# musket-ml/segmentation_training_pipeline

Measured on AMD Instinct MI355X. Metric: images/sec U-Net/ResNet34 512x512 bs16 training step, higher is better.
Workload: dtype bf16; 1 GPU; U-Net/ResNet34 512x512x3 1-class, batch 16 per GPU, BCE+Dice, Adam, on-device augment S1 (BASELINE.json configs[1]); global_batch=16, parallelism=dp1, hipgraph=True

## Files before the change

segmentation_training_pipeline_amd/csrc/conv_common.h:

```cpp
#pragma once
#include <type_traits>
#include "common.h"
#include <cstdlib>

struct ConvArgs {
  const char* src0;
  const char* src1;
  const char* weight;
  const char* residual;
  const float* bias;
  char* dst0;
  char* dst1;
  int N, Hs0, Ws0, Hv, Wv, C0, C1, Ctot, mode;
  int KH, KW, stride, pad, Ho, Wo, Cout, Cd0, Cd1;
  int acc0, acc1, relu;
  int K, P, HoWo, wrows;
  int ntile_m, ntile_n;
  uint32_t bytes0, bytes1, bytesw;
  float* stats;
  int stat_slots;
  BnBack bnb;
  BnBack pbn;
  FastDiv divC, divKW, divHoWo, divWo, divNtm;
  int zperm, zPc, zH2W2, zW2, zcpt;
  FastDiv divPc, divH2W2, divW2, divCpt;
  const char* weight_up;
  uint32_t byteswu;
  int upc, ucpt0, ucpt1;
  FastDiv divU0, divU1;
  const char* fold_src;
  const char* fold_weight;
  int fold_cpt;
  uint32_t bytes_fold, bytesw_fold;
  int no_rm;
  int ep_generic;
  int sum2x2;
  float* sg_out;
  unsigned* sg_cnt;
  int sg_G;
  int d2s;
};

__device__ __forceinline__ void stats_store(const ConvArgs& a, size_t idx, float v) {
  if (a.sg_out) __hip_atomic_store(a.stats + idx, v, __ATOMIC_RELAXED, __HIP_MEMORY_SCOPE_AGENT);
  else a.stats[idx] = v;
}
template <int NT>
__device__ __forceinline__ void stats_group_finish(const ConvArgs& a, int Cs, int cout0, int nch, int tile_m, int tile_n, int ntile, int tid,
                                                   unsigned* word) {
  if (!a.sg_out) return;
  const int G = a.sg_G, g = tile_n / G, ngroups = (ntile + G - 1) / G;
  const int members = (ntile - g * G) < G ? (ntile - g * G) : G;
  unsigned* const cnt = a.sg_cnt + (size_t)tile_m * ngroups + g;
  asm volatile("s_waitcnt vmcnt(0)" ::: "memory");
  __syncthreads();
  if (tid == 0) *word = __hip_atomic_fetch_add(cnt, 1u, __ATOMIC_RELAXED, __HIP_MEMORY_SCOPE_AGENT);
  __syncthreads();
  if (*word != (unsigned)(members - 1)) return;
  if (tid == 0) __hip_atomic_store(cnt, 0u, __ATOMIC_RELAXED, __HIP_MEMORY_SCOPE_AGENT);
  for (int r = tid; r < 2 * nch; r += NT) {
    const int stat = r / nch, ch = cout0 + (r - stat * nch);
    if (ch >= Cs) continue;
    const float* col = a.stats + ((size_t)stat * Cs + ch) * ntile + (size_t)g * G;
    float v[16];
#pragma unroll
    for (int j = 0; j < 16; ++j) v[j] = j < members ? __hip_atomic_load(col + j, __ATOMIC_RELAXED, __HIP_MEMORY_SCOPE_AGENT) : 0.f;
    float sum = v[0];
#pragma unroll
    for (int j = 1; j < 16; ++j) sum += v[j];
    a.sg_out[((size_t)stat * Cs + ch) * ngroups + g] = sum;
  }
}
static inline int stats_group_size(int cols) {
  if (cols <= 128) return 0;
// ... 419 lines not shown
  if (p->Cd0 <= 0 || p->Cd0 > p->Cout || (p->Cd0 < p->Cout && (!p->dst1 || (p->Cd0 & 3) || ((p->Cout - p->Cd0) & 3))))
    return STP_E_BADARG;
  if (p->N <= 0 || p->Ho <= 0 || p->Wo <= 0 || p->Cout <= 0 || p->KH <= 0 || p->KW <= 0 || p->stride <= 0) return STP_E_BADARG;
  a.src0 = (const char*)p->src0; a.src1 = (const char*)p->src1; a.weight = (const char*)p->weight;
  a.residual = (const char*)p->residual; a.bias = p->bias; a.dst0 = (char*)p->dst0; a.dst1 = (char*)p->dst1;
  a.N = p->N; a.Hs0 = p->Hs0; a.Ws0 = p->Ws0; a.Hv = p->Hv; a.Wv = p->Wv; a.C0 = p->C0; a.C1 = p->C1;
  a.Ctot = p->C0 + p->C1; a.mode = p->src0_mode;
  a.KH = p->KH; a.KW = p->KW; a.stride = p->stride; a.pad = p->pad; a.Ho = p->Ho; a.Wo = p->Wo;
  a.Cout = p->Cout; a.Cd0 = p->Cd0; a.Cd1 = p->Cout - p->Cd0;
  a.acc0 = p->accumulate0; a.acc1 = p->accumulate1; a.relu = p->relu;
  a.K = p->KH * p->KW * a.Ctot;
  const int64_t P = (int64_t)p->N * p->Ho * p->Wo;
  if (P >= (1ll << 31)) return STP_E_BADARG;
  a.P = (int)P; a.HoWo = p->Ho * p->Wo; a.wrows = round_up(p->Cout, 16);
  a.divC = make_fastdiv((uint32_t)a.Ctot); a.divKW = make_fastdiv((uint32_t)a.KW);
  a.divHoWo = make_fastdiv((uint32_t)(p->Ho * p->Wo)); a.divWo = make_fastdiv((uint32_t)p->Wo);
  const int64_t lim = 1ll << 31;
  const int64_t b0 = (int64_t)p->N * p->Hs0 * p->Ws0 * p->C0 * sz;
  const int64_t b1 = (int64_t)p->N * p->Hv * p->Wv * p->C1 * sz;
  const int64_t bw = (int64_t)a.wrows * a.K * sz;
  a.bytes0 = (uint32_t)(b0 < lim ? b0 : 0); a.bytes1 = (uint32_t)(b1 < lim ? b1 : 0); a.bytesw = (uint32_t)(bw < lim ? bw : 0);
  a.ntile_m = a.ntile_n = 0;
  a.zperm = 0;
  a.weight_up = (const char*)p->weight_up; a.byteswu = 0; a.upc = 0; a.ucpt0 = a.ucpt1 = 1;
  a.fold_src = a.fold_weight = nullptr; a.fold_cpt = 0; a.bytes_fold = a.bytesw_fold = 0;
  {
    static const int no_rm = (getenv("STP_IGEMM_RM") && atoi(getenv("STP_IGEMM_RM")) == 0) ? 1 : 0;
    a.no_rm = no_rm;
    static const int ep_generic = (getenv("STP_EPILOGUE_SPECIAL") && atoi(getenv("STP_EPILOGUE_SPECIAL")) == 0) ? 1 : 0;
    a.ep_generic = ep_generic;
  }
  a.stats = p->stats_partial;
  a.stat_slots = p->stats_slots;
  if (a.stats && ((p->Cout & 3) || (p->Cd0 != p->Cout && !p->dst_sum2x2))) return STP_E_BADARG;
  a.sum2x2 = p->dst_sum2x2 ? 1 : 0;
  a.sg_out = nullptr; a.sg_cnt = nullptr; a.sg_G = 0;
  a.d2s = p->s2d_dgrad ? 1 : 0;
  if (p->stats_group > 1) {
    if (!p->stats_group_out || !p->stats_group_counters || !a.stats || a.stat_slots || p->stats_group > 16 || (p->stats_group & (p->stats_group - 1)))
      return STP_E_BADARG;
    a.sg_out = p->stats_group_out; a.sg_cnt = p->stats_group_counters; a.sg_G = p->stats_group;
  }
  if (a.stat_slots && (!a.stats || (a.stat_slots & (a.stat_slots - 1)) || a.stat_slots > 64)) return STP_E_BADARG;
  a.bnb.x = (const char*)p->bnb_x; a.bnb.mean = p->bnb_mean; a.bnb.rstd = p->bnb_rstd; a.bnb.gamma = p->bnb_gamma;
  a.bnb.beta = p->bnb_beta; a.bnb.relu = p->bnb_relu;
  a.pbn.x = nullptr; a.pbn.mean = p->src_bn_mean; a.pbn.rstd = p->src_bn_rstd; a.pbn.gamma = p->src_bn_gamma; a.pbn.beta = p->src_bn_beta;
  a.pbn.relu = p->src_bn_relu;
  *c4_out = c4;
  *ut_out = 0;
  if (!c4 && b0 < lim && b1 < lim && bw < lim) {
    if ((a.Ctot % ke == 0) && (a.C0 % ke == 0)) *ut_out = 1;
    else if (a.C1 == 0 && (ke % a.Ctot == 0)) *ut_out = 2;
  }
  return STP_OK;
}
```

segmentation_training_pipeline_amd/csrc/conv_halo.hip:

```cpp
#include "conv_common.h"
#include <cstdlib>
#include <type_traits>

#define STP_OOB 0x80000000u
#define HALO_NWST 4
#if defined(STP_TIMING_REAL)
#define STP_CLOCK() __builtin_amdgcn_s_memrealtime()
#else
#define STP_CLOCK() __builtin_amdgcn_s_memtime()
#endif


__device__ __forceinline__ void wait_vmcnt_n(int n) {
  switch (n) {
    case 0: wait_vmcnt<0>(); break;
    case 1: wait_vmcnt<1>(); break;
    case 2: wait_vmcnt<2>(); break;
    case 3: wait_vmcnt<3>(); break;
    case 4: wait_vmcnt<4>(); break;
    case 5: wait_vmcnt<5>(); break;
    case 6: wait_vmcnt<6>(); break;
    case 7: wait_vmcnt<7>(); break;
    case 8: wait_vmcnt<8>(); break;
    case 9: wait_vmcnt<9>(); break;
// ... 572 lines not shown
#pragma unroll
      for (int dx = 0; dx < 3; ++dx)
#pragma unroll
        for (int kc = 0; kc < 4; ++kc) b_lane[dx][kc] += d;
    }
    if (!grp_b) __builtin_amdgcn_s_barrier();
  }
  STP_STAMP(2);

  epilogue_rm<TH, BM, WM, WN, EP>(a, acc, smem, n, y0, x0, cout0, tile_n, wm, wn, lane, tid, wave);
#if defined(STP_TIMING)
  asm volatile("s_waitcnt vmcnt(0)" ::: "memory");
  STP_STAMP(3);
  if (tid == 0)
    for (int i = 0; i < 4; ++i) tdbg[(size_t)blockIdx.x * 4 + i] = tstamp[i];
#endif
#endif
}

#define HALO_MIN_WAVES(TH, BM) ((TH) == 16 && (BM) == 64 ? 4 : 1)
template <int TH, int BM, int WM, int WN, int EP>
__global__ __launch_bounds__(512, HALO_MIN_WAVES(TH, BM)) void conv_halo_kernel(const ConvArgs a) { conv_halo_body<TH, BM, WM, WN, EP, false, false>(a); }
template <int TH, int BM, int WM, int WN, int EP>
__global__ __launch_bounds__(512, HALO_MIN_WAVES(TH, BM)) void conv_halo_pbn_kernel(const ConvArgs a) { conv_halo_body<TH, BM, WM, WN, EP, true, false>(a); }
template <int TH, int BM, int WM, int WN, int EP>
__global__ __launch_bounds__(512, 1) void conv_halo_r6_kernel(const ConvArgs a) { conv_halo_body<TH, BM, WM, WN, EP, false, false, 9, false, 6>(a); }
template <int TH, int BM, int WM, int WN, int EP>
__global__ __launch_bounds__(512, HALO_MIN_WAVES(TH, BM)) void conv_halo2_kernel(const ConvArgs a) { conv_halo_body<TH, BM, WM, WN, EP, false, true>(a); }
template <int TH, int BM, int WM, int WN, int EP>
__global__ __launch_bounds__(512, HALO_MIN_WAVES(TH, BM)) void conv_halo_fold1_kernel(const ConvArgs a) { conv_halo_body<TH, BM, WM, WN, EP, false, true, 9, true>(a); }
template <int TH, int BM, int WM, int WN, int EP>
__global__ __launch_bounds__(512, HALO_MIN_WAVES(TH, BM)) void conv_halo_s2d_kernel(const ConvArgs a) { conv_halo_body<TH, BM, WM, WN, EP, false, true, 4>(a); }

#if !defined(STP_P64_STAGGER)
#define STP_P64_STAGGER 4
#endif
template <int TH, int BM, int WM, int WN, int EP>
__global__ __launch_bounds__(256, 2) void conv_halo_p64_kernel(const ConvArgs a_in) {
  static_assert(TH == 8 && BM == 64 && WM == 2 && WN == 2 && EP <= 2, "the 64 -> 64 form");
#if defined(__HIP_DEVICE_COMPILE__)
#if defined(STP_TIMING)
  ConvArgs a = a_in;
  unsigned long long* const tdbg = reinterpret_cast<unsigned long long*>(const_cast<float*>(a_in.bias));
  a.bias = nullptr;
  unsigned long long tsum[4] = {0, 0, 0, 0}, tlast = STP_CLOCK();
  const unsigned long long tfirst = tlast;
#define P64_LAP(i) { const unsigned long long now_ = STP_CLOCK(); tsum[i] += now_ - tlast; tlast = now_; }
#else
  const ConvArgs& a = a_in;
#define P64_LAP(i)
#endif
  typedef bf16_t T;
  constexpr int NTH = 256;
  constexpr int TW = 16, HWD = TW + 2, HH = TH + 2, NHP = HH * HWD;
  constexpr int SROWS = (NHP + 7) / 8 * 8, SLAB = SROWS * 128;
  constexpr int NPASS = (SROWS + 31) / 32;
  constexpr int RW = TH / WN, TN = RW / 2;
  constexpr int PF = 2;
  extern __shared__ __attribute__((aligned(16))) char smem[];
  char* const stage = smem + 2 * SLAB;
  const int tid = threadIdx.x, lane = tid & 63;
  const int wave = __builtin_amdgcn_readfirstlane(tid >> 6);
  const int wm = wave / WN, wn = wave % WN;
  const int l15 = lane & 15, l31 = lane & 31, l4b = (lane >> 4) & 1, l5 = lane >> 5;
  const int ntile = a.ntile_n, nwg = gridDim.x;
  const int wg = xcd_remap(blockIdx.x, nwg);
// ... 145 lines not shown
    done = true;
  }
  hipLaunchKernelGGL(kern, dim3(a.ntile_m * a.ntile_n), dim3(512), lds, s, a);
  STP_LAUNCH_CHECK();
  return STP_OK;
}

template <int TH, int BM, int WM, int WN>
static int launch_halo(ConvArgs& a, hipStream_t s) {
  if (a.sum2x2) return launch_halo_ep<TH, BM, WM, WN, 3>(a, s);
  if (a.bnb.x) return launch_halo_ep<TH, BM, WM, WN, 2>(a, s);
  if (a.stats) return launch_halo_ep<TH, BM, WM, WN, 1>(a, s);
  return launch_halo_ep<TH, BM, WM, WN, 0>(a, s);
}

static bool halo2_enabled() {
  static const bool on = !(getenv("STP_HALO2") && atoi(getenv("STP_HALO2")) == 0);
  return on;
}
static bool halo_src_ok(const stp_conv_params* p) {
  const bool direct = p->src0_mode == STP_SRC_DIRECT && p->Hs0 == p->Hv && p->Ws0 == p->Wv;
  if (direct && p->C1 == 0) return true;
  const bool up2 = p->src0_mode == STP_SRC_NEAREST2X && p->Hs0 * 2 == p->Hv && p->Ws0 * 2 == p->Wv;
  return halo2_enabled() && (direct || up2) && (p->C1 == 0 || (p->src1 && (p->C1 % 64) == 0)) && !p->src_bn_mean && !p->bnb_x && !p->dst_sum2x2 &&
         p->Cd0 == p->Cout;
}
static bool halo_s2d_ok(const stp_conv_params* p) {
  static const bool on = !(getenv("STP_S2D") && atoi(getenv("STP_S2D")) == 0);
  return on && p && p->s2d_dgrad && p->dtype == STP_H16 && p->KH == 2 && p->KW == 2 && p->stride == 1 && p->pad == 0 && p->src0_mode == STP_SRC_DIRECT &&
         p->Hs0 == p->Hv && p->Ws0 == p->Wv && p->Ho == p->Hv && p->Wo == p->Wv && (p->Wo % 16) == 0 && (p->Ho % 8) == 0 && p->C0 >= 64 &&
         (p->C0 % 64) == 0 && (p->C1 == 0 || (p->src1 && p->fold_weight && (p->C1 % 64) == 0)) && (p->Cout % 128) == 0 && p->Cd0 == p->Cout && !p->dst1 &&
         !p->dst_sum2x2 && !p->stats_slots && !p->src_bn_mean && !p->bias && !p->relu && !p->residual && !p->accumulate1;
}
static bool halo_fold1_ok(const stp_conv_params* p) {
  static const bool on = !(getenv("STP_FOLD1") && atoi(getenv("STP_FOLD1")) == 0);
  return on && p->fold_src && p->fold_weight && p->fold_C >= 64 && (p->fold_C % 64) == 0 && p->C1 == 0 && p->src0_mode == STP_SRC_DIRECT &&
         !p->src_bn_mean && !p->dst_sum2x2 && !p->dst1 && p->Cd0 == p->Cout && !p->bias && !p->relu && !p->residual;
}
static bool halo_p64_ok(const stp_conv_params* p) {
  static const bool on = !(getenv("STP_HALO_P64") && atoi(getenv("STP_HALO_P64")) == 0);
  return on && p->C0 == 64 && p->C1 == 0 && p->Cout == 64 && p->Cd0 == 64 && !p->dst1 && p->src0_mode == STP_SRC_DIRECT && !p->fold_src && !p->s2d_dgrad &&
         !p->src_bn_mean && !p->dst_sum2x2 && (p->Ho % 8) == 0;
}
static int halo_cus() {
  static int n = 0;
  if (!n) {
    int dev = 0, v = 0;
    if (hipGetDevice(&dev) != hipSuccess || hipDeviceGetAttribute(&v, hipDeviceAttributeMultiprocessorCount, dev) != hipSuccess || v <= 0) v = 256;
    n = v;
  }
  return n;
}
template <int EP>
static int launch_halo_p64_ep(ConvArgs& a, hipStream_t s) {
  constexpr int TH = 8, NHP = (TH + 2) * 18, SROWS = (NHP + 7) / 8 * 8;
  const size_t lds = (size_t)2 * SROWS * 128 + (size_t)TH * 16 * (64 * 4 + 16);
  static_assert(2 * SROWS * 128 + TH * 16 * (64 * 4 + 16) >= 9 * 64 * 128, "the weight image fits the workgroup's LDS");
  a.ntile_m = 1;
  a.ntile_n = a.N * (a.Ho / TH) * (a.Wo / 16);
  auto kern = conv_halo_p64_kernel<8, 64, 2, 2, EP>;
  static bool attr_set = false;
  if (!attr_set) {
    if (hipFuncSetAttribute(reinterpret_cast<const void*>(kern), hipFuncAttributeMaxDynamicSharedMemorySize, 160 * 1024) != hipSuccess) return STP_E_LAUNCH;
    attr_set = true;
  }
  const int slots = 2 * halo_cus();
  const int nwg = a.ntile_n < slots ? a.ntile_n : slots;
  hipLaunchKernelGGL(kern, dim3(nwg), dim3(256), lds, s, a);
  STP_LAUNCH_CHECK();
  return STP_OK;
}
static int launch_halo_p64(ConvArgs& a, hipStream_t s) {
  if (a.sum2x2 || a.pbn.mean) return STP_E_BADARG;
  if (a.bnb.x) return launch_halo_p64_ep<2>(a, s);
  if (a.stats) return launch_halo_p64_ep<1>(a, s);
  return launch_halo_p64_ep<0>(a, s);
}

static bool halo_shape_ok(const stp_conv_params* p) {
  if (p && p->s2d_dgrad) return halo_s2d_ok(p);
  if (p && p->fold_src && !halo_fold1_ok(p)) return false;
  return p && p->dtype == STP_H16 && p->KH == 3 && p->KW == 3 && p->stride == 1 && p->pad == 1 && halo_src_ok(p) &&
         p->C0 >= 64 && (p->C0 % 64) == 0 && p->Ho == p->Hv && p->Wo == p->Wv &&
         (p->Wo % 16) == 0 && (p->Ho % 8) == 0 && (p->Cout % 16) == 0 && p->Cout >= 64 && !p->stats_slots &&
         (!p->dst_sum2x2 || (p->bnb_x && (p->Cd0 % 64) == 0 && !p->bias && !p->relu && !p->residual &&
                             (p->Cd0 == p->Cout || (p->dst1 && p->Cd0 < p->Cout)))) &&
         (p->Cd0 % 8) == 0 &&
         (!p->src_bn_mean || (p->src_bn_rstd && p->C0 <= 512));
}

static int halo_auto(const stp_conv_params* p) {
  if (!halo_shape_ok(p)) return -1;
  {
    static const int force = getenv("STP_HALO_FORCE") ? atoi(getenv("STP_HALO_FORCE")) : -1;
    if (force >= 0 && force < 4 && (p->Ho % (force == 0 || force == 2 ? 16 : 8)) == 0) return force;
  }
  const int64_t px16 = (p->Ho % 16) == 0 ? (int64_t)p->N * (p->Ho / 16) * (p->Wo / 16) : 0;
  const int64_t px8 = (int64_t)p->N * (p->Ho / 8) * (p->Wo / 16);
  if (p->s2d_dgrad) {
    const int ct2 = ceil_div(p->Cout, 128);
    if (px16 * ct2 >= 256) return 0;
    return px8 * ct2 >= 192 ? 1 : -1;
  }
  if (p->C1 > 0 || p->src0_mode != STP_SRC_DIRECT) {
    static const bool c64 = !(getenv("STP_HALO2_64") && atoi(getenv("STP_HALO2_64")) == 0);
    if (p->Cout <= 64 && !c64) return -1;
  }
  if (p->fold_src && p->C0 == 64) {
    return px8 * ceil_div(p->Cout, 64) >= 512 ? 3 : -1;
  }
  if (p->C0 == 64 && p->C1 == 0) {
    if (p->Cout > 64 && (p->Ho % 32) == 0 && (int64_t)p->N * (p->Ho / 32) * (p->Wo / 16) * ceil_div(p->Cout, 64) >= 512) return 4;
    static const int p64 = getenv("STP_HALO_P64") ? atoi(getenv("STP_HALO_P64")) : 0;
    if (p64 == 1 && halo_p64_ok(p) && px8 >= 4 * halo_cus()) return 5;
    static const int v4 = getenv("STP_HALO_64V4") ? atoi(getenv("STP_HALO_64V4")) : 0;
    if (v4 == 1 && (p->Ho % 32) == 0 && (int64_t)p->N * (p->Ho / 32) * (p->Wo / 16) >= 512) return 4;
    if (px16 * ceil_div(p->Cout, 64) >= 512) return 2;
    if (px8 * ceil_div(p->Cout, 64) >= 512) return 3;
    return -1;
  }
  const int ct = ceil_div(p->Cout, 128);
  if (p->Cout > 64 && px16 * ct >= 256) return 0;
  if (p->Cout > 64 && px8 * ct >= 192) return 1;
  if (px8 * ceil_div(p->Cout, 64) >= 192) return 3;
  return -1;
}

extern "C" int stp_conv2d_halo_variant(const stp_conv_params* p) {
  if (!p) return -1;
  int v = -1;
  if (p->tile >= STP_TILE_HALO && p->tile < STP_TILE_HALO + HALO_NCFG) {
    v = p->tile - STP_TILE_HALO;
    if (!halo_shape_ok(p) || (p->Ho % HALO_CFGS[v].th) || (v == 4 && (p->C0 != 64 || p->C1)) || (p->s2d_dgrad && v > 1) || (v == 5 && !halo_p64_ok(p))) return -1;
  } else if (p->tile == 0) {
    v = halo_auto(p);
  }
  if (v >= 0 && p->dst_sum2x2 && (p->Cd0 % HALO_CFGS[v].bm)) return -1;
  return v;
}

extern "C" int stp_conv2d_halo_tiles(const stp_conv_params* p, int variant) {
  return p->N * (p->Ho / HALO_CFGS[variant].th) * (p->Wo / 16);
}

extern "C" int stp_conv2d_halo(const stp_conv_params* p, int variant, void* stream) {
  if (variant < 0 || variant >= HALO_NCFG || !halo_shape_ok(p) || (p->Ho % HALO_CFGS[variant].th) || (variant == 4 && (p->C0 != 64 || p->C1)) ||
      (p->s2d_dgrad && variant > 1) || (variant == 5 && !halo_p64_ok(p))) return STP_E_BADARG;
  ConvArgs a;
  bool c4;
  int ut;
  const int rc = fill_args(p, a, &c4, &ut);
  if (rc != STP_OK) return rc;
  if (ut != 1) return STP_E_BADARG;
  if (a.bnb.x && (!a.stats || !a.bnb.mean || !a.bnb.rstd || p->relu || p->residual)) return STP_E_BADARG;
  if (a.sum2x2 && (!a.bnb.x || (p->Cd0 % HALO_CFGS[variant].bm))) return STP_E_BADARG;
  if (!p->s2d_dgrad && p->fold_src) {
    if (!halo_fold1_ok(p)) return STP_E_BADARG;
    const int64_t bf = (int64_t)p->N * p->Hv * p->Wv * p->fold_C * 2, bwf = (int64_t)round_up(p->Cout, 16) * p->fold_C * 2;
    if (bf >= (1ll << 31) || bwf >= (1ll << 31)) return STP_E_BADARG;
    a.src1 = (const char*)p->fold_src; a.C1 = p->fold_C; a.Ctot = a.C0 + a.C1; a.bytes1 = (uint32_t)bf;
    a.fold_weight = (const char*)p->fold_weight; a.bytesw_fold = (uint32_t)bwf;
  }
  if (p->s2d_dgrad) {
    const int64_t rows = round_up(p->Cout / 4, 16), bw = rows * 9 * p->C0 * 2, bf = rows * (int64_t)p->C1 * 2;
    if (bw >= (1ll << 31) || bf >= (1ll << 31) || (p->C1 > 0 && !p->fold_weight)) return STP_E_BADARG;
    a.bytesw = (uint32_t)bw;
    a.fold_weight = p->C1 > 0 ? (const char*)p->fold_weight : nullptr;
    a.bytesw_fold = (uint32_t)bf;
  }
  const_cast<stp_conv_params*>(p)->stats_tiles = stp_conv2d_halo_tiles(p, variant) * (p->s2d_dgrad ? 4 : 1);
  hipStream_t s = (hipStream_t)stream;
  switch (variant) {
    case 0: return launch_halo<16, 128, 2, 4>(a, s);
    case 1: return launch_halo<8, 128, 2, 4>(a, s);
    case 2: return launch_halo<16, 64, 1, 8>(a, s);
    case 3: return launch_halo<8, 64, 2, 4>(a, s);
    case 4: return launch_halo<32, 64, 1, 8>(a, s);
    case 5: return launch_halo_p64(a, s);
    default: return STP_E_BADARG;
  }
}
```

segmentation_training_pipeline_amd/csrc/conv_igemm.hip:

```cpp
#include "conv_common.h"
#include <cstdlib>

#define STP_OOB 0x80000000u

template <typename T, int BM, int BN, int WM, int WN, int STAGES, bool UNI, bool UPC = false, bool ZP = false>
__global__ __launch_bounds__(256) void conv_igemm_ut_kernel(const ConvArgs a) {
  static_assert(!UPC || ZP, "the class-collapsed layers use the parity-class pixel order");
  static_assert(WM * WN == 4 && BM % 16 == 0 && BN % 32 == 0 && STAGES >= 2, "config");
#if defined(__HIP_DEVICE_COMPILE__)
  constexpr int SZ = (int)sizeof(T);
  constexpr int VEC = Elem<T>::VEC;
  constexpr int KE = 128 / SZ;
  constexpr int TM = BM / WM / 16, TN = BN / WN / 16;
  constexpr int RA = (BM + 31) / 32, RB = BN / 32;
  constexpr int STAGE = (BM + BN) * 128;
  constexpr int L = RA + RB;
  constexpr int DUMP = STAGES * STAGE;

  extern __shared__ __attribute__((aligned(16))) char smem[];
  const int tid = threadIdx.x, lane = tid & 63;
  const int wave = __builtin_amdgcn_readfirstlane(tid >> 6);
  const int wm = wave / WN, wn = wave % WN;
  const int r0 = tid >> 3;
  const int lslot = (tid & 7) ^ (r0 & 7);
// ... 645 lines not shown
}

extern "C" int stp_conv2d(const stp_conv_params* p, void* stream) {
  if (p && p->stats_group > 1 && p->stats_group != stp_conv2d_stats_group_for(p)) return STP_E_BADARG;
  if (p && (p->tile == 0 || p->tile == STP_TILE_SC)) {
    if (stp_conv2d_sc_eligible(p)) return stp_conv2d_sc(p, stream);
    if (p->tile == STP_TILE_SC) return STP_E_BADARG;
  }
  if (p && (p->tile == 0 || p->tile == STP_TILE_SCW)) {
    if (stp_conv2d_scw_eligible(p)) return stp_conv2d_scw(p, stream);
    if (p->tile == STP_TILE_SCW) return STP_E_BADARG;
  }
  if (p && (p->tile == 0 || p->tile == STP_TILE_SCN)) {
    if (stp_conv2d_scn_eligible(p)) return stp_conv2d_scn(p, stream);
    if (p->tile == STP_TILE_SCN) return STP_E_BADARG;
  }
  if (p && ((p->tile == 0 && s64_auto()) || p->tile == STP_TILE_S64)) {
    if (stp_conv2d_s64_eligible(p)) return stp_conv2d_s64(p, stream);
    if (p->tile == STP_TILE_S64) return STP_E_BADARG;
  }
  if (p && (p->tile == 0 || p->tile == STP_TILE_STEM)) {
    if (stp_conv2d_stem_eligible(p)) return stp_conv2d_stem(p, stream);
    if (p->tile == STP_TILE_STEM) return STP_E_BADARG;
  }
  if (p && (p->tile == 0 || p->tile == STP_TILE_PW)) {
    if (stp_conv2d_pw_eligible(p)) return stp_conv2d_pw(p, stream);
    if (p->tile == STP_TILE_PW) return STP_E_BADARG;
  }
  {
    const int hv = halo_variant_for(p);
    if (hv >= 0) return stp_conv2d_halo(p, hv, stream);
    if (p && p->tile >= STP_TILE_HALO) return STP_E_BADARG;
    if (p && (p->s2d_dgrad || (p->fold_src && p->src0_mode != STP_SRC_ZEROINS2X))) return STP_E_BADARG;
  }
  ConvArgs a;
  bool c4;
  int ut;
  const int rc = fill_args(p, a, &c4, &ut);
  if (rc != STP_OK) return rc;
  if (p->dst_sum2x2 || p->src_bn_mean) return STP_E_BADARG;
  if (a.bnb.x && (!a.stats || !a.bnb.mean || !a.bnb.rstd || p->relu || p->residual)) return STP_E_BADARG;
  int tile = p->tile ? p->tile : auto_tile(a, ut);
  if (c4 && tile != 2 && tile != 5) tile = 2;
  hipStream_t s = (hipStream_t)stream;
  const_cast<stp_conv_params*>(p)->stats_tiles = ceil_div(a.P, tile_pixels(tile));
  {
    const int ke = p->dtype == STP_H16 ? 64 : 32;
    if (zperm_applies(a, tile, ut)) {
      a.zperm = 1;
      a.zPc = a.P / 4; a.zH2W2 = (a.Ho / 2) * (a.Wo / 2); a.zW2 = a.Wo / 2; a.zcpt = a.Ctot / ke;
      a.divPc = make_fastdiv((uint32_t)a.zPc); a.divH2W2 = make_fastdiv((uint32_t)a.zH2W2); a.divW2 = make_fastdiv((uint32_t)a.zW2);
      a.divCpt = make_fastdiv((uint32_t)a.zcpt);
    }
    if (p->fold_src) {
      if (!a.zperm || !fold_geometry_ok(a) || !p->fold_weight || p->fold_C != a.C0) return STP_E_BADARG;
      const int64_t bf = (int64_t)a.N * a.Hs0 * a.Ws0 * a.C0 * (p->dtype == STP_H16 ? 2 : 4), bwf = (int64_t)a.wrows * a.C0 * (p->dtype == STP_H16 ? 2 : 4);
      if (bf >= (1ll << 31) || bwf >= (1ll << 31)) return STP_E_BADARG;
      a.fold_src = (const char*)p->fold_src; a.fold_weight = (const char*)p->fold_weight; a.fold_cpt = a.C0 / ke;
      a.bytes_fold = (uint32_t)bf; a.bytesw_fold = (uint32_t)bwf;
    }
  }
  {
    static const bool upc_on = !(getenv("STP_UPCOLLAPSE") && atoi(getenv("STP_UPCOLLAPSE")) == 0);
    const int ke = p->dtype == STP_H16 ? 64 : 32;
    const bool uni_tile = (tile >= 64 && tile < 96) || tile == 128 + 5;
    if (upc_on && p->weight_up && a.mode == STP_SRC_NEAREST2X && ut == 1 && uni_tile && a.stride == 1 && a.KH == 3 && a.KW == 3 && a.pad == 1 &&
// ... 17 lines not shown
```

segmentation_training_pipeline_amd/graph.py:

```python
import os
import ctypes as C
from collections import OrderedDict

import numpy as np
import torch

from . import _lib, ops

_TD = {"bf16": torch.bfloat16, "fp16": torch.float16, "fp32": torch.float32}


class StpShapeError(ValueError):
    pass


def _rup(a, b):
    return (a + b - 1) // b * b


class DT(object):
    __slots__ = ("name", "N", "H", "W", "C", "buf", "grad", "_grad_ready", "grad_writes", "needs_grad", "gradC", "meta")

    def __init__(self, name, N, H, W, Cn, buf=None, needs_grad=False):
        self.name, self.N, self.H, self.W, self.C = name, N, H, W, Cn
# ... 633 lines not shown
        out = self._new(name, Ho, Wo, Cout, x_ng or s_ng or w.trainable or (residual is not None and residual.needs_grad))
        out.gradC = CoutB
        if bias:
            self._bn_ws_c = max(self._bn_ws_c, CoutB)
        self._use(x, src1, residual)
        wp = _lib.WgradParams()
        wp.N, wp.Hs0, wp.Ws0, wp.Hv, wp.Wv, wp.C0, wp.C1 = self.N, x.H, x.W, Hv, Wv, C0, C1
        src_mode = ops.SRC_NEAREST2X if upsample else (ops.SRC_ZEROINS2X if transpose else ops.SRC_DIRECT)
        wp.src0_mode = src_mode
        wp.KH, wp.KW, wp.stride, wp.pad, wp.Ho, wp.Wo, wp.Cout = k, KWp, stride, pad, Ho, Wo, CoutB
        wp.accumulate, wp.dtype, wp.splits = 0, self.cdt, 0
        if self.training and w.trainable:
            self._wg_ws_bytes = max(self._wg_ws_bytes, int(self.lib.stp_conv2d_wgrad_workspace_bytes(C.byref(wp))))
        if self.dry:
            return out
        rows_f, rows_b = _rup(Cout, 16), _rup(Cinp, 16)
        wf = self._alloc((rows_f * k * KWp * Cinp,))
        need_dgrad = self.training and (x_ng or s_ng) and not stem
        wb = self._alloc((rows_b * k * k * CoutB,)) if need_dgrad else None
        out.meta["wb"] = wb
        wsrc = self._pptr(w)
        if param_cols is not None:
            w.pending_slices += 1
            wm = self._alloc((Cout * Cin_master,), torch.float32)
            self._emit(self.prep, "stp_copy_cols_f32", wm.data_ptr(), Cin_master, wsrc + 4 * int(param_cols[0]), int(param_cols[1]), Cout, Cin_master, 0)
            wsrc = wm.data_ptr()
        out.meta["w_master"] = (wsrc, Cout, Cin_master, k)
        self._prep_layers.append((wsrc, wf.data_ptr(), wb.data_ptr() if wb is not None else None,
                                  Cout, k, k, Cin_master, KWp, Cinp, CoutB))
        p = ops.conv_params(x.buf, wf, out.buf, N=self.N, Hs0=x.H, Ws0=x.W, Hv=Hv, Wv=Wv, C0=C0, C1=C1,
                            src1=src1.buf if src1 is not None else None,
                            mode=src_mode, KH=k, KW=KWp, stride=stride, pad=pad,
                            Ho=Ho, Wo=Wo, Cout=Cout, dtype=self.cdt, residual=residual.buf if residual is not None else None)
        w4 = None
        if (upsample and src1 is not None and k == 3 and KWp == 3 and stride == 1 and pad == 1 and Cinp == Cin_master == C0 + C1
                and os.environ.get("STP_UPCOLLAPSE", "1") != "0" and not self.lib.stp_conv2d_scn_eligible(C.byref(p))
                and int(self.lib.stp_conv2d_halo_variant(C.byref(p))) < 0):
            wup = self._alloc((rows_f * 16 * C0,))
            self._upc_layers.append((self._pptr(w), wup.data_ptr(), Cout, rows_f, C0, C0 + C1))
            p.weight_up = wup.data_ptr()
            if need_dgrad and x_ng and C0 % 16 == 0 and os.environ.get("STP_UPCOLLAPSE_BWD", "0") == "1":
                w4 = self._alloc((C0 * 16 * CoutB,))
                self._upc4_layers.append((self._pptr(w), w4.data_ptr(), Cout, CoutB, C0, C0 + C1))
        if (self.training and x.meta.get("apply_rec") is not None and src1 is None and residual is None and not transpose and not stem
                and self.lib.stp_conv2d_sc_eligible(C.byref(p)) and (not w.trainable or self.lib.stp_wgrad_sc_eligible(C.byref(wp)))):
            x.meta["sc_consumers"].append((p, wp))
        elif (self.training and self.fuse_bn_halo and x.meta.get("apply_rec") is not None and src1 is None and not transpose and not stem
                and not upsample and self.lib.stp_conv2d_halo_variant(C.byref(p)) >= 0):
            x.meta["halo_consumers"].append((p, wp, (not w.trainable) or int(self.lib.stp_conv2d_wgrad_kernel_id(C.byref(wp))) in (2, 3)))
        if b is not None:
            p.bias = self._pptr(b)
        if relu:
            if CoutB != Cout:
                raise StpShapeError("%s: a fused ReLU needs Cout to be a multiple of %d" % (name, self.vec))
            p.relu = 1
        if bn_stats and self.training and self.slot_arena is not None and self.N * Ho * Wo <= self.bn_slots_max_rows:
            sp, sn = self._slots(Cout)
            p.stats_partial, p.stats_slots = sp, sn
            out.meta["stats_slots"] = (sp, sn)
        elif bn_stats and self.training:
            nfl = int(self.lib.stp_conv2d_stats_floats(C.byref(p)))
            st = self._alloc((max(nfl, 4),), torch.float32)
            p.stats_partial = st.data_ptr()
            out.meta["stats"] = (st, p)
            out.meta["stats_table"] = self._group_stats(p, st, Cout)
        flops = 2.0 * self.N * Ho * Wo * Cout * k * k * Cin_master / (4.0 if transpose else 1.0)
        if flops_as is not None:
            flops = float(flops_as)
        self._emit_conv(self.fwd, p, {"layer": name, "pass": "fwd", "flops": flops, "tile": int(self.lib.stp_conv2d_tile_for(C.byref(p))),
                                      "src2": bool(C1 or upsample)})
        if not self.training:
            return out

        def back():
            if not out.needs_grad or not out.grad_ready:
                return
            dy = out.grad
            rows = out.rows
            if relu:
                self._before_inplace_write(dy)
                self._emit(self.bwd, "stp_relu_bwd", out.buf.data_ptr(), dy.data_ptr(), rows * out.gradC, self.cdt)
            if self._side_lag_join or not self._side_groups_only:
                self._mark(self.bwd, "join")
                self._side_reads.clear()
                self._side_groups_only = True
            if residual is not None and residual.needs_grad:
                if not residual.grad_ready and residual.gradC == out.gradC:
                    residual.grad = dy
                    residual.grad_ready = True
                else:
                    self._emit(self.bwd, "stp_add_inplace", self._gradbuf(residual).data_ptr(), dy.data_ptr(),
                               rows * out.gradC, self.cdt)
            if w.trainable:
                padded = stem or CoutB != Cout
                gcols = None
                if padded:
                    dwp = self._alloc((CoutB * k * KWp * Cinp,), torch.float32)
                    wp.dw = dwp.data_ptr()
                elif param_cols is not None:
                    gcols = self._alloc((Cout * Cin_master,), torch.float32)
                    wp.dw = gcols.data_ptr()
                else:
                    wp.dw = self._gptr(w)
# ... 885 lines not shown
```

Before: 2509 images/sec.

## Add forward stride-2 space-to-depth halo conv kernel fused with 1x1 shortcut

Adds a new halo kernel for forward 3x3 stride-2 convolutions that stages the four parity classes of the input in LDS and runs nine tap steps through MFMA. In the graph builder it can also fold the preceding 1x1 stride-2 shortcut conv into the same launch, either as extra output tiles or merged into the same tile with a second accumulator. This removes the separate shortcut launch and a second read of the input. The cost is a complex new kernel with LDS-DMA pipelining and extra restrictions on shapes and stats, and it only applies to ResNet downsampling blocks. A helper script for comparing numerical dumps is also added.

Result: no change. 2519 images/sec, median of 6 (+0.4%).

```diff
diff --git a/scratch/r08/compare_dumps.py b/scratch/r08/compare_dumps.py
--- /dev/null
+++ b/scratch/r08/compare_dumps.py
@@ -0,0 +1,14 @@
+import os
+import sys
+
+import numpy as np
+
+a_dir, b_dir = sys.argv[1], sys.argv[2]
+for f in sorted(os.listdir(a_dir)):
+    if not f.endswith(".npy"):
+        continue
+    a, b = np.load(os.path.join(a_dir, f)).astype(np.float64), np.load(os.path.join(b_dir, f)).astype(np.float64)
+    d = np.abs(a - b)
+    rng = float(np.abs(a).max()) or 1.0
+    print("%-32s n %9d  range %.6g  max|d| %.4g  mean|d| %.4g  mean|d| / (range * 2^-8) %.3f  identical %.4f"
+          % (f[:-4], a.size, rng, d.max(), d.mean(), d.mean() / (rng * 2.0 ** -8), float((d == 0).mean())))
diff --git a/segmentation_training_pipeline_amd/csrc/conv_common.h b/segmentation_training_pipeline_amd/csrc/conv_common.h
--- a/segmentation_training_pipeline_amd/csrc/conv_common.h
+++ b/segmentation_training_pipeline_amd/csrc/conv_common.h
@@ -39,7 +39,9 @@
   unsigned* sg_cnt;
   int sg_G;
   int d2s;
+  int s2f;
 };
+static inline bool stp_is_fwd_fold(const stp_conv_params* p) { return p && p->fold_weight && !p->fold_src && !p->s2d_dgrad; }
 
 __device__ __forceinline__ void stats_store(const ConvArgs& a, size_t idx, float v) {
   if (a.sg_out) __hip_atomic_store(a.stats + idx, v, __ATOMIC_RELAXED, __HIP_MEMORY_SCOPE_AGENT);
@@ -525,10 +527,11 @@
   }
   a.stats = p->stats_partial;
   a.stat_slots = p->stats_slots;
-  if (a.stats && ((p->Cout & 3) || (p->Cd0 != p->Cout && !p->dst_sum2x2))) return STP_E_BADARG;
+  if (a.stats && ((p->Cout & 3) || (p->Cd0 != p->Cout && !p->dst_sum2x2 && !stp_is_fwd_fold(p)))) return STP_E_BADARG;
   a.sum2x2 = p->dst_sum2x2 ? 1 : 0;
   a.sg_out = nullptr; a.sg_cnt = nullptr; a.sg_G = 0;
   a.d2s = p->s2d_dgrad ? 1 : 0;
+  a.s2f = 0;
   if (p->stats_group > 1) {
     if (!p->stats_group_out || !p->stats_group_counters || !a.stats || a.stat_slots || p->stats_group > 16 || (p->stats_group & (p->stats_group - 1)))
       return STP_E_BADARG;
diff --git a/segmentation_training_pipeline_amd/csrc/conv_halo.hip b/segmentation_training_pipeline_amd/csrc/conv_halo.hip
--- a/segmentation_training_pipeline_amd/csrc/conv_halo.hip
+++ b/segmentation_training_pipeline_amd/csrc/conv_halo.hip
@@ -628,6 +628,226 @@
 template <int TH, int BM, int WM, int WN, int EP>
 __global__ __launch_bounds__(512, HALO_MIN_WAVES(TH, BM)) void conv_halo_s2d_kernel(const ConvArgs a) { conv_halo_body<TH, BM, WM, WN, EP, false, true, 4>(a); }
 
+__host__ __device__ constexpr int s2f_dy(int j) { return (0x1bc >> j) & 1; }
+__host__ __device__ constexpr int s2f_dx(int j) { return (0x1ea >> j) & 1; }
+__host__ __device__ constexpr int s2f_buf(int j) { return j < 4 ? 0 : j < 6 ? 1 : j < 8 ? 2 : 3; }
+__host__ __device__ constexpr int s2f_tap(int j) { return j == 0 ? 0 : j == 1 ? 2 : j == 2 ? 6 : j == 3 ? 8 : j == 4 ? 3 : j == 5 ? 5 : j == 6 ? 1 : j == 7 ? 7 : 4; }
+__host__ __device__ constexpr int s2f_pcls(int j, int slot) {
+  return j == 0 ? (slot == 0 ? 2 : -1) : j == 1 ? 3 : j == 2 ? (slot == 0 ? 3 : -1) : j == 3 ? -1 : j == 4 ? 0 : j == 5 ? (slot == 0 ? 0 : -1) :
+         j == 6 ? 1 : j == 7 ? (slot == 0 ? 1 : -1) : 2;
+}
+__host__ __device__ constexpr int s2f_ppass(int j, int slot) { return (j == 1 || j == 4 || j == 6 || j == 8) ? slot : 2; }
+__host__ __device__ constexpr bool s2f_pnext(int j) { return j >= 4; }
+
+template <int TH, int BM, int WM, int WN, int EP, bool MERGE>
+__device__ __forceinline__ void conv_halo_s2f_body(const ConvArgs& a) {
+  static_assert(TH == 8 && BM == 128 && WM == 2 && WN == 4 && EP <= 1, "the forward space-to-depth form: 8 x 16 pixels x 128 channels");
+#if defined(__HIP_DEVICE_COMPILE__)
+  constexpr int TW = 16, HWD = TW + 2, HH = TH + 2, NHP = HH * HWD;
+  constexpr int NPASS = (NHP + 63) / 64;
+  static_assert(NPASS == 3, "the pass schedule above");
+  constexpr int SROWS = (NHP + 7) / 8 * 8, SLAB = SROWS * 128;
+  constexpr int WSTAGE = BM * 128, LW = BM / 64;
+  constexpr int CW = BM / WM, RW = TH / WN, TM = CW / 32, TN = RW / 2;
+  constexpr int OFF_W = 4 * SLAB;
+  static_assert(TN == 1 && LW + 2 <= TM * TN * 4, "one LDS-DMA instruction per MFMA at most");
+
+  extern __shared__ __attribute__((aligned(16))) char smem[];
+  const int tid = threadIdx.x, lane = tid & 63;
+  const int wave = __builtin_amdgcn_readfirstlane(tid >> 6);
+  const int wm = wave / WN, wn = wave % WN;
+  const int l15 = lane & 15, l31 = lane & 31, l4b = (lane >> 4) & 1, l5 = lane >> 5;
+
+  const int bid = xcd_remap(blockIdx.x, a.ntile_m * a.ntile_n);
+  const int tile_n = bid / a.ntile_m, tile_m = bid - tile_n * a.ntile_m;
+  const int tx_n = a.Wo / TW, ty_n = a.Ho / TH;
+  const int n = tile_n / (tx_n * ty_n), trem = tile_n - n * (tx_n * ty_n);
+  const int ty = trem / tx_n, tx = trem - ty * tx_n;
+  const int y0 = ty * TH, x0 = tx * TW, cout0 = tile_m * BM;
+  const bool sc_tile = !MERGE && cout0 >= a.Cd0;
+  constexpr int NJ = MERGE ? 10 : 9;
+
+  const __amdgpu_buffer_rsrc_t rsw = __builtin_amdgcn_make_buffer_rsrc((void*)(sc_tile ? a.fold_weight : a.weight), 0, sc_tile ? a.bytesw_fold : a.bytesw, 0x00020000);
+  const __amdgpu_buffer_rsrc_t rs0 = __builtin_amdgcn_make_buffer_rsrc((void*)a.src0, 0, a.bytes0, 0x00020000);
+  const __amdgpu_buffer_rsrc_t rsw2 = __builtin_amdgcn_make_buffer_rsrc((void*)(MERGE ? a.fold_weight : a.weight), 0, MERGE ? a.bytesw_fold : a.bytesw, 0x00020000);
+
+  const int prow = tid >> 3, pslot = tid & 7;
+  uint32_t soff[NPASS];
+#pragma unroll
+  for (int i = 0; i < NPASS; ++i) {
+    const int hp = i * 64 + prow;
+    const int hy = hp / HWD, hx = hp - hy * HWD;
+    const int ya = y0 - 1 + hy, xb = x0 - 1 + hx;
+    const bool ok = hp < NHP && hy <= TH && hx <= TW && ya >= 0 && xb >= 0;
+    const uint32_t ch = (uint32_t)((pslot ^ ((hx >> 1) & 7)) * 8);
+    soff[i] = ok ? (((uint32_t)(n * a.Hv + 2 * ya) * (uint32_t)a.Wv + (uint32_t)(2 * xb)) * (uint32_t)a.C0 + ch) * 2u : STP_OOB;
+  }
+  const uint32_t colb = (uint32_t)a.C0 * 2u, rowb = (uint32_t)a.Wv * colb;
+  const uint32_t cls_off[4] = {rowb + colb, colb, rowb, 0u};
+  const uint32_t wpitch = sc_tile ? colb : 9u * colb;
+  const int wrow0 = sc_tile ? cout0 - a.Cd0 : cout0, wrows = sc_tile ? a.Cd1 : a.Cd0;
+  uint32_t woff[LW];
+#pragma unroll
+  for (int i = 0; i < LW; ++i) {
+    const int r = wrow0 + i * 64 + prow;
+    woff[i] = r < wrows ? (uint32_t)r * wpitch + (uint32_t)((pslot ^ ((prow >> 1) & 7)) * 8) * 2u : STP_OOB;
+  }
+  uint32_t woff2[MERGE ? LW : 1];
+  if constexpr (MERGE) {
+#pragma unroll
+    for (int i = 0; i < LW; ++i) {
+      const int r = cout0 + i * 64 + prow;
+      woff2[i] = r < a.Cd1 ? (uint32_t)r * colb + (uint32_t)((pslot ^ ((prow >> 1) & 7)) * 8) * 2u : STP_OOB;
+    }
+  }
+  const int nchunk = a.C0 >> 6;
+  const int nstep = sc_tile ? nchunk : nchunk * NJ;
+
+  auto pass_on = [&](int p) { return (p * 64 + wave * 8) < SROWS; };
+  auto issue_slab_pass = [&](int cls, int q, int p) {
+    if (!pass_on(p)) return;
+    __builtin_amdgcn_raw_ptr_buffer_load_lds(rs0, (__attribute__((address_space(3))) void*)(smem + cls * SLAB + (p * 64 + wave * 8) * 128), 16, soff[p],
+                                             cls_off[cls] + (uint32_t)q * 128u, 0, 0);
+  };
+  auto issue_weight_piece = [&](int i, int st, uint32_t col, bool on, bool second = false) {
+    if (MERGE && second)
+      __builtin_amdgcn_raw_ptr_buffer_load_lds(rsw2, (__attribute__((address_space(3))) void*)(smem + OFF_W + st * WSTAGE + (i * 64 + wave * 8) * 128), 16,
+                                               on ? woff2[MERGE ? i : 0] : STP_OOB, col, 0, 0);
+    else
+      __builtin_amdgcn_raw_ptr_buffer_load_lds(rsw, (__attribute__((address_space(3))) void*)(smem + OFF_W + st * WSTAGE + (i * 64 + wave * 8) * 128), 16,
+                                               on ? woff[i] : STP_OOB, col, 0, 0);
+  };
+
+  uint32_t a_lane[4], b_lane[2][4];
+#pragma unroll
+  for (int kc = 0; kc < 4; ++kc) {
+    a_lane[kc] = (uint32_t)(OFF_W + (wm * CW + l31) * 128 + (((kc * 2 + l5) ^ ((l31 >> 1) & 7)) << 4));
+#pragma unroll
+    for (int dx = 0; dx < 2; ++dx) {
+      const int hx = l15 + dx;
+      b_lane[dx][kc] = (uint32_t)(((wn * RW + l4b) * HWD + hx) * 128 + (((kc * 2 + l5) ^ ((hx >> 1) & 7)) << 4));
+    }
+  }
+
+  f32x16 acc[TM][TN], acc2[MERGE ? TM : 1][TN];
+#pragma unroll
+  for (int i = 0; i < TM; ++i)
+#pragma unroll
+    for (int e = 0; e < 16; ++e) {
+      acc[i][0][e] = 0.f;
+      if (MERGE) acc2[MERGE ? i : 0][0][e] = 0.f;
+    }
+
+  if (sc_tile) {
+#pragma unroll
+    for (int q = 0; q < 4; ++q)
+      if (q < nchunk) {
+#pragma unroll
+        for (int p = 0; p < NPASS; ++p) {
+          if (!pass_on(p)) continue;
+          __builtin_amdgcn_raw_ptr_buffer_load_lds(rs0, (__attribute__((address_space(3))) void*)(smem + q * SLAB + (p * 64 + wave * 8) * 128), 16, soff[p],
+                                                   (uint32_t)q * 128u, 0, 0);
+        }
+      }
+#pragma unroll
+    for (int t = 0; t < 3; ++t)
+#pragma unroll
+      for (int i = 0; i < LW; ++i) issue_weight_piece(i, t, (uint32_t)t * 128u, t < nstep);
+  } else {
+#pragma unroll
+    for (int p = 0; p < NPASS; ++p) issue_slab_pass(0, 0, p);
+#pragma unroll
+    for (int p = 0; p < NPASS; ++p) issue_slab_pass(1, 0, p);
+    issue_slab_pass(2, 0, 0);
+    issue_slab_pass(2, 0, 1);
+#pragma unroll
+    for (int t = 0; t < 3; ++t)
+#pragma unroll
+      for (int i = 0; i < LW; ++i) issue_weight_piece(i, t, (uint32_t)s2f_tap(t) * colb, true);
+  }
+
+  const bool grp_b = wave >= 4;
+  wait_vmcnt<2 * LW>();
+  __builtin_amdgcn_s_barrier();
+  if (grp_b) __builtin_amdgcn_s_barrier();
+
+  u32x4 fa[4][TM], fb[4];
+  int wst = 0;
+  auto kstep = [&](auto& ac, const int buf, const int dy, const int dx, const int young, const uint32_t col3, const bool won, const bool w2, auto&& slab_piece) __attribute__((always_inline)) {
+    const uint32_t so = (uint32_t)(wst * WSTAGE);
+#pragma unroll
+    for (int kc = 0; kc < 4; ++kc) {
+      fb[kc] = *reinterpret_cast<const u32x4*>(smem + b_lane[dx][kc] + buf * SLAB + dy * (HWD * 128));
+#pragma unroll
+      for (int i = 0; i < TM; ++i) fa[kc][i] = *reinterpret_cast<const u32x4*>(smem + a_lane[kc] + so + i * 4096);
+    }
+    asm volatile("s_waitcnt lgkmcnt(0)" ::: "memory");
+    wait_vmcnt_n(young);
+    __builtin_amdgcn_s_barrier();
+    __builtin_amdgcn_sched_barrier(0);
+    __builtin_amdgcn_s_setprio(1);
+    const int st3 = (wst + 3) & 3;
+    int piece = 0;
+#pragma unroll
+    for (int kc = 0; kc < 4; ++kc)
+#pragma unroll
+      for (int i = 0; i < TM; ++i) {
+        ac[i][0] = mfma16_32x32x16(fa[kc][i], fb[kc], ac[i][0]);
+        __builtin_amdgcn_sched_barrier(0);
+        if (piece < LW) issue_weight_piece(piece, st3, col3, won, w2);
+        else if (piece < LW + 2) slab_piece(piece - LW);
+        __builtin_amdgcn_sched_barrier(0);
+        ++piece;
+      }
+    __builtin_amdgcn_s_setprio(0);
+    __builtin_amdgcn_sched_barrier(0);
+    __builtin_amdgcn_s_barrier();
+    wst = (wst + 1) & 3;
+  };
+
+  if (sc_tile) {
+    for (int q = 0; q < nchunk; ++q)
+      kstep(acc, q, 1, 1, LW, (uint32_t)(q + 3) * 128u, q + 3 < nstep, false, [](int) {});
+  } else {
+    for (int q = 0; q < nchunk; ++q) {
+      const bool last = q + 1 == nchunk;
+#pragma unroll
+      for (int j = 0; j < NJ; ++j) {
+        const int jp = j == 0 ? NJ - 1 : j - 1;
+        int np = 0;
+#pragma unroll
+        for (int sl = 0; sl < 2; ++sl)
+          if (jp < 9 && s2f_pcls(jp, sl) >= 0 && pass_on(s2f_ppass(jp, sl)) && !(j == 0 ? q == 0 : (s2f_pnext(jp) && last))) ++np;
+        const int j3 = (j + 3) % NJ, q3 = q + (j + 3) / NJ;
+        const uint32_t col3 = (j3 == 9 ? 0u : (uint32_t)s2f_tap(j3) * colb) + (uint32_t)q3 * 128u;
+        auto slabs = [&](int sl) {
+          if (j >= 9 || s2f_pcls(j, sl) < 0 || (s2f_pnext(j) && last)) return;
+          issue_slab_pass(s2f_pcls(j, sl), q + (s2f_pnext(j) ? 1 : 0), s2f_ppass(j, sl));
+        };
+        if (MERGE && j == 9) kstep(acc2, 3, 1, 1, LW + np, col3, q3 < nchunk, j3 == 9, slabs);
+        else kstep(acc, s2f_buf(j), s2f_dy(j), s2f_dx(j), LW + np, col3, q3 < nchunk, j3 == 9, slabs);
+      }
+    }
+  }
+  if (!grp_b) __builtin_amdgcn_s_barrier();
+
+  if (sc_tile) {
+    epilogue_rm<TH, BM, WM, WN, 0>(a, acc, smem, n, y0, x0, cout0, tile_n, wm, wn, lane, tid, wave);
+  } else {
+    ConvArgs am = a;
+    am.Cout = a.Cd0;
+    epilogue_rm<TH, BM, WM, WN, EP>(am, acc, smem, n, y0, x0, cout0, tile_n, wm, wn, lane, tid, wave);
+    if constexpr (MERGE) {
+      ConvArgs as = a;
+      as.stats = nullptr;
+      epilogue_rm<TH, BM, WM, WN, 0>(as, acc2, smem, n, y0, x0, cout0 + a.Cd0, tile_n, wm, wn, lane, tid, wave);
+    }
+  }
+#endif
+}
+template <int TH, int BM, int WM, int WN, int EP, bool FWD, bool MERGE = false>
+__global__ __launch_bounds__(512, 1) void conv_halo_s2d_kernel(const ConvArgs a) { static_assert(FWD, "forward form"); conv_halo_s2f_body<TH, BM, WM, WN, EP, MERGE>(a); }
+
 #if !defined(STP_P64_STAGGER)
 #define STP_P64_STAGGER 4
 #endif
@@ -839,6 +1059,18 @@
          (p->C0 % 64) == 0 && (p->C1 == 0 || (p->src1 && p->fold_weight && (p->C1 % 64) == 0)) && (p->Cout % 128) == 0 && p->Cd0 == p->Cout && !p->dst1 &&
          !p->dst_sum2x2 && !p->stats_slots && !p->src_bn_mean && !p->bias && !p->relu && !p->residual && !p->accumulate1;
 }
+static bool halo_s2f_ok(const stp_conv_params* p) {
+  static const bool on = !(getenv("STP_S2D_FWD") && atoi(getenv("STP_S2D_FWD")) == 0);
+  static const bool fold_on = !(getenv("STP_FOLD_SC_FWD") && atoi(getenv("STP_FOLD_SC_FWD")) == 0);
+  if (!on || !p || p->s2d_dgrad || p->dtype != STP_H16 || p->KH != 3 || p->KW != 3 || p->stride != 2 || p->pad != 1 || p->src0_mode != STP_SRC_DIRECT ||
+      p->Hs0 != p->Hv || p->Ws0 != p->Wv || p->Hv != 2 * p->Ho || p->Wv != 2 * p->Wo || (p->Wo % 16) || (p->Ho % 8) || p->C0 < 64 || (p->C0 % 64) || p->C1 ||
+      p->src1 || p->fold_src || p->dst_sum2x2 || p->stats_slots || p->src_bn_mean || p->bias || p->relu || p->residual || p->bnb_x || p->accumulate0 ||
+      p->accumulate1 || p->Cd0 < 128 || (p->Cd0 % 128))
+    return false;
+  if (stp_is_fwd_fold(p))
+    return fold_on && p->dst1 && p->fold_C >= 128 && (p->fold_C % 128) == 0 && p->Cd0 + p->fold_C == p->Cout && p->C0 <= 256;
+  return !p->dst1 && p->Cd0 == p->Cout;
+}
 static bool halo_fold1_ok(const stp_conv_params* p) {
   static const bool on = !(getenv("STP_FOLD1") && atoi(getenv("STP_FOLD1")) == 0);
   return on && p->fold_src && p->fold_weight && p->fold_C >= 64 && (p->fold_C % 64) == 0 && p->C1 == 0 && p->src0_mode == STP_SRC_DIRECT &&
@@ -877,6 +1109,25 @@
   STP_LAUNCH_CHECK();
   return STP_OK;
 }
+template <int EP>
+static int launch_halo_s2f(ConvArgs& a, hipStream_t s) {
+  constexpr int TH = 8, BM = 128, NHP = (TH + 2) * 18, SROWS = (NHP + 7) / 8 * 8;
+  constexpr size_t lds = (size_t)4 * SROWS * 128 + (size_t)HALO_NWST * BM * 128;
+  static_assert(lds <= 160 * 1024 && lds >= (size_t)TH * 16 * (BM * 4 + 16), "the LDS of a CU; the epilogue's staged tile fits");
+  a.ntile_n = a.N * (a.Ho / TH) * (a.Wo / 16);
+  static const bool merge_on = !(getenv("STP_S2D_FWD_MERGE") && atoi(getenv("STP_S2D_FWD_MERGE")) == 0);
+  const bool merge = merge_on && a.fold_weight && a.Cd1 == a.Cd0 && (int64_t)a.ntile_n * (a.Cd0 / BM) >= 192;
+  a.ntile_m = (merge ? a.Cd0 : a.Cout) / BM;
+  auto kern = merge ? conv_halo_s2d_kernel<TH, BM, 2, 4, EP, true, true> : conv_halo_s2d_kernel<TH, BM, 2, 4, EP, true, false>;
+  static bool attr_set[2] = {false, false};
+  if (!attr_set[merge]) {
+    if (hipFuncSetAttribute(reinterpret_cast<const void*>(kern), hipFuncAttributeMaxDynamicSharedMemorySize, 160 * 1024) != hipSuccess) return STP_E_LAUNCH;
+    attr_set[merge] = true;
+  }
+  hipLaunchKernelGGL(kern, dim3(a.ntile_m * a.ntile_n), dim3(512), lds, s, a);
+  STP_LAUNCH_CHECK();
+  return STP_OK;
+}
 static int launch_halo_p64(ConvArgs& a, hipStream_t s) {
   if (a.sum2x2 || a.pbn.mean) return STP_E_BADARG;
   if (a.bnb.x) return launch_halo_p64_ep<2>(a, s);
@@ -886,6 +1137,8 @@
 
 static bool halo_shape_ok(const stp_conv_params* p) {
   if (p && p->s2d_dgrad) return halo_s2d_ok(p);
+  if (p && p->stride == 2) return halo_s2f_ok(p);
+  if (stp_is_fwd_fold(p)) return false;
   if (p && p->fold_src && !halo_fold1_ok(p)) return false;
   return p && p->dtype == STP_H16 && p->KH == 3 && p->KW == 3 && p->stride == 1 && p->pad == 1 && halo_src_ok(p) &&
          p->C0 >= 64 && (p->C0 % 64) == 0 && p->Ho == p->Hv && p->Wo == p->Wv &&
@@ -898,6 +1151,7 @@
 
 static int halo_auto(const stp_conv_params* p) {
   if (!halo_shape_ok(p)) return -1;
+  if (p->stride == 2) return (stp_is_fwd_fold(p) && (int64_t)p->N * (p->Ho / 8) * (p->Wo / 16) * (p->Cout / 128) >= 192) ? 1 : -1;
   {
     static const int force = getenv("STP_HALO_FORCE") ? atoi(getenv("STP_HALO_FORCE")) : -1;
     if (force >= 0 && force < 4 && (p->Ho % (force == 0 || force == 2 ? 16 : 8)) == 0) return force;
@@ -939,6 +1193,7 @@
   if (p->tile >= STP_TILE_HALO && p->tile < STP_TILE_HALO + HALO_NCFG) {
     v = p->tile - STP_TILE_HALO;
     if (!halo_shape_ok(p) || (p->Ho % HALO_CFGS[v].th) || (v == 4 && (p->C0 != 64 || p->C1)) || (p->s2d_dgrad && v > 1) || (v == 5 && !halo_p64_ok(p))) return -1;
+    if (p->stride == 2 && v != 1) return -1;
   } else if (p->tile == 0) {
     v = halo_auto(p);
   }
@@ -952,7 +1207,7 @@
 
 extern "C" int stp_conv2d_halo(const stp_conv_params* p, int variant, void* stream) {
   if (variant < 0 || variant >= HALO_NCFG || !halo_shape_ok(p) || (p->Ho % HALO_CFGS[variant].th) || (variant == 4 && (p->C0 != 64 || p->C1)) ||
-      (p->s2d_dgrad && variant > 1) || (variant == 5 && !halo_p64_ok(p))) return STP_E_BADARG;
+      (p->s2d_dgrad && variant > 1) || (variant == 5 && !halo_p64_ok(p)) || (p->stride == 2 && variant != 1)) return STP_E_BADARG;
   ConvArgs a;
   bool c4;
   int ut;
@@ -977,6 +1232,15 @@
   }
   const_cast<stp_conv_params*>(p)->stats_tiles = stp_conv2d_halo_tiles(p, variant) * (p->s2d_dgrad ? 4 : 1);
   hipStream_t s = (hipStream_t)stream;
+  if (p->stride == 2) {
+    const int64_t bw = (int64_t)round_up(p->Cd0, 16) * 9 * p->C0 * 2, bf = (int64_t)round_up(p->Cout - p->Cd0, 16) * p->C0 * 2;
+    if (bw >= (1ll << 31) || bf >= (1ll << 31) || a.bnb.x || a.sum2x2 || a.pbn.mean) return STP_E_BADARG;
+    a.s2f = 1;
+    a.bytesw = (uint32_t)bw;
+    a.fold_weight = stp_is_fwd_fold(p) ? (const char*)p->fold_weight : nullptr;
+    a.bytesw_fold = (uint32_t)bf;
+    return a.stats ? launch_halo_s2f<1>(a, s) : launch_halo_s2f<0>(a, s);
+  }
   switch (variant) {
     case 0: return launch_halo<16, 128, 2, 4>(a, s);
     case 1: return launch_halo<8, 128, 2, 4>(a, s);
diff --git a/segmentation_training_pipeline_amd/csrc/conv_igemm.hip b/segmentation_training_pipeline_amd/csrc/conv_igemm.hip
--- a/segmentation_training_pipeline_amd/csrc/conv_igemm.hip
+++ b/segmentation_training_pipeline_amd/csrc/conv_igemm.hip
@@ -701,6 +701,7 @@
     if (hv >= 0) return stp_conv2d_halo(p, hv, stream);
     if (p && p->tile >= STP_TILE_HALO) return STP_E_BADARG;
     if (p && (p->s2d_dgrad || (p->fold_src && p->src0_mode != STP_SRC_ZEROINS2X))) return STP_E_BADARG;
+    if (stp_is_fwd_fold(p)) return STP_E_BADARG;
   }
   ConvArgs a;
   bool c4;
diff --git a/segmentation_training_pipeline_amd/graph.py b/segmentation_training_pipeline_amd/graph.py
--- a/segmentation_training_pipeline_amd/graph.py
+++ b/segmentation_training_pipeline_amd/graph.py
@@ -689,6 +689,17 @@
                             src1=src1.buf if src1 is not None else None,
                             mode=src_mode, KH=k, KW=KWp, stride=stride, pad=pad,
                             Ho=Ho, Wo=Wo, Cout=Cout, dtype=self.cdt, residual=residual.buf if residual is not None else None)
+        fwd_fold = None
+        if (fold_shortcut is not None and stride == 2 and k == 3 and KWp == 3 and pad == 1 and src1 is None and not upsample and not transpose
+                and not stem and residual is None and not bias and not relu and os.environ.get("STP_HALO", "1") != "0"
+                and self.fwd and self.fwd[-1] is fold_shortcut.meta.get("fwd_rec")
+                and not (x.meta.get("sc_consumers") or x.meta.get("halo_consumers"))):
+            pf = ops.conv_params(x.buf, wf, out.buf, N=self.N, Hs0=x.H, Ws0=x.W, Hv=Hv, Wv=Wv, C0=C0, mode=src_mode, KH=k, KW=KWp, stride=stride,
+                                 pad=pad, Ho=Ho, Wo=Wo, Cout=Cout + fold_shortcut.C, Cd0=Cout, dst1=fold_shortcut.buf, dtype=self.cdt)
+            pf.fold_weight, pf.fold_C = fold_shortcut.meta["wf"].data_ptr(), fold_shortcut.C
+            if int(self.lib.stp_conv2d_halo_variant(C.byref(pf))) >= 0:
+                p = pf
+                fwd_fold = self.fwd.pop()
         w4 = None
         if (upsample and src1 is not None and k == 3 and KWp == 3 and stride == 1 and pad == 1 and Cinp == Cin_master == C0 + C1
                 and os.environ.get("STP_UPCOLLAPSE", "1") != "0" and not self.lib.stp_conv2d_scn_eligible(C.byref(p))
@@ -720,12 +731,17 @@
             st = self._alloc((max(nfl, 4),), torch.float32)
             p.stats_partial = st.data_ptr()
             out.meta["stats"] = (st, p)
-            out.meta["stats_table"] = self._group_stats(p, st, Cout)
+            out.meta["stats_table"] = self._group_stats(p, st, int(p.Cout))
+            if fwd_fold is not None and out.meta["stats_table"][0] is not st:
+                raise StpShapeError("%s: the forward fold has no group-level pre-reduction of its sums" % name)
         flops = 2.0 * self.N * Ho * Wo * Cout * k * k * Cin_master / (4.0 if transpose else 1.0)
         if flops_as is not None:
             flops = float(flops_as)
-        self._emit_conv(self.fwd, p, {"layer": name, "pass": "fwd", "flops": flops, "tile": int(self.lib.stp_conv2d_tile_for(C.byref(p))),
-                                      "src2": bool(C1 or upsample)})
+        fmeta = {"layer": name, "pass": "fwd", "flops": flops, "tile": int(self.lib.stp_conv2d_tile_for(C.byref(p))), "src2": bool(C1 or upsample)}
+        if fwd_fold is not None:
+            fmeta.update(flops=flops + fwd_fold[3]["flops"], s2d=True, fold_fwd=fold_shortcut.name)
+        self._emit_conv(self.fwd, p, fmeta)
+        out.meta["fwd_rec"], out.meta["wf"] = self.fwd[-1], wf
         if not self.training:
             return out
 
```
